# AVianEco/Softspoken

Measured on AMD Instinct MI355X. Metric: audio-seconds processed/sec (whole node), 16 kHz mono, higher is better.
Workload: dtype f16x2

## Files before the change

### softspoken_amd/build.py

```python
from __future__ import annotations

import os
import subprocess
import sys

HERE = os.path.dirname(os.path.abspath(__file__))
CSRC = os.path.join(HERE, "csrc")
OBJ = os.path.join(CSRC, "_obj")
LIB = os.path.join(HERE, "libsoftspoken_hip.so")
DEV_LIB = os.path.join(HERE, "libsoftspoken_hip_dev.so")
SOURCES = ["conv2.hip", "conv2_ups.hip", "conv4.hip", "conv4_ups.hip", "conv1s.hip", "frontend.hip", "heads.hip", "weights.hip", "engine.hip", "host.hip", "abi.hip", "stream.hip", "separate.hip"]
HEADERS = [os.path.join(CSRC, h) for h in ("kernels.h", "engine.h", "dsp.h", "mfma_util.h", "conv4_forms.h")] + [os.path.join(os.path.dirname(HERE), "include", "softspoken.h")]
FLAGS = ["-O3", "--offload-arch=gfx950", "-fPIC", "-std=c++17", "-Wno-unused-value"]
EXTRA_FLAGS = {"frontend.hip": ["-fno-slp-vectorize"], "conv4.hip": ["-fno-slp-vectorize"], "conv4_ups.hip": ["-fno-slp-vectorize"],
               "conv1s.hip": ["-fno-slp-vectorize"]}
DEV_SOURCES = ("conv2.hip", "conv2_ups.hip", "conv4.hip", "conv4_ups.hip", "conv1s.hip", "frontend.hip", "engine.hip", "weights.hip", "abi.hip", "separate.hip")
JITTER_LIB = DEV_LIB


def _hipcc():
    for cand in (os.environ.get("HIPCC"), "/opt/rocm/bin/hipcc"):
        if cand and os.path.exists(cand):
            return cand
    return "hipcc"


def _stale(target, deps):
    if not os.path.exists(target):
        return True
    t = os.path.getmtime(target)
# ... 36 lines not shown
```

### softspoken_amd/csrc/conv1s.hip

```cpp
#include "kernels.h"
#include "mfma_util.h"
#include <algorithm>
#include <type_traits>

namespace ss {

static constexpr int kH = 128, kW = 256, kC = 32;
static constexpr int kStrips = 9, kStripCols = 30;
static constexpr int kBank = 9 * 2 * 1024;
static constexpr int kS1Waves = 8;
static constexpr int kFPitch = 36;
static constexpr int kMaxRows = 32;
static constexpr int kFPatch = (kMaxRows + 5) * kFPitch;

__device__ __forceinline__ float s1_from_left(float v) {
    return __builtin_bit_cast(float, __builtin_amdgcn_update_dpp(0, __builtin_bit_cast(int, v), 0x138, 0xf, 0xf, true));
}
__device__ __forceinline__ float s1_from_right(float v) {
    return __builtin_bit_cast(float, __builtin_amdgcn_update_dpp(0, __builtin_bit_cast(int, v), 0x130, 0xf, 0xf, true));
}

struct S1Row { u32x4 f[2][2]; };

template <bool TRACK>
__global__ __launch_bounds__(64 * kS1Waves) __attribute__((amdgpu_waves_per_eu(2, 2)))
void conv1_stream_kernel(ConvArgs a, int rows_per_unit, int total_units) {
    extern __shared__ __attribute__((aligned(16))) char smem[];
// ... 258 lines not shown
        }
        if (k < rows_per_unit) {
            row_step(y0 + k, H0, H1, H2);
            if (k + 1 < rows_per_unit) row_step(y0 + k + 1, H1, H2, H0);
        }
    }
#ifdef SS_DEVBUILD
    if (a.stamps && lane == 0) {
        uint32_t* p = (uint32_t*)a.stamps + ((size_t)blockIdx.x * kS1Waves + wave) * 16;
        for (int i = 0; i < 7; ++i) p[i] = st_sum[i];
    }
#endif
    if (((ovf & 0x7fff7fffu) + 0x04000400u) & 0x80008000u) atomicOr(a.range_flag, 1);
}

struct S16Row { u32x4 f[2][2]; };

__device__ __forceinline__ f32x4 s16_mfma(const u32x4& a, const u32x4& b, const f32x4& c) {
    return __builtin_amdgcn_mfma_f32_16x16x32_f16(__builtin_bit_cast(f16x8, a), __builtin_bit_cast(f16x8, b), c, 0, 0, 0);
}
__device__ __forceinline__ int s16_shr1(int v) { return __builtin_amdgcn_update_dpp(0, v, 0x111, 0xf, 0xf, true); }
__device__ __forceinline__ int s16_shl1(int v) { return __builtin_amdgcn_update_dpp(0, v, 0x101, 0xf, 0xf, true); }
__device__ __forceinline__ float s16_shr1f(float v) { return __int_as_float(s16_shr1(__float_as_int(v))); }
__device__ __forceinline__ float s16_shl1f(float v) { return __int_as_float(s16_shl1(__float_as_int(v))); }

static constexpr int kFPatch16 = (kMaxRows + 6) * kFPitch;

template <bool TRACK>
__global__ __launch_bounds__(64 * kS1Waves) __attribute__((amdgpu_waves_per_eu(2, 2)))
void conv1_stream16_kernel(ConvArgs a, int rows_per_unit, int total_units) {
    extern __shared__ __attribute__((aligned(16))) char smem[];
    char* sW = smem;
    char* sK = smem + 2 * kBank;
    char* sPrev = sK + 4 * 1024;
    float* sF = (float*)(sPrev + kS1Waves * 2048);

    const int tid = threadIdx.x, lane = tid & 63, wave = __builtin_amdgcn_readfirstlane(tid >> 6);
    const int g = lane >> 4, c = lane & 15;
    for (int p = tid; p < 2 * kBank / 16; p += 64 * kS1Waves) *(u32x4*)(sW + p * 16) = *(const u32x4*)((const char*)a.wpk + (size_t)p * 16);
    u32x4 wf1[2];
// ... 126 lines not shown
                    Hn.f[t][0] = u32x4{ph[0][0], ph[0][1], ph[1][0], ph[1][1]};
                    Hn.f[t][1] = u32x4{pl[0][0], pl[0][1], pl[1][0], pl[1][1]};
                    if (edge_strip) {
#pragma unroll
                        for (int pq = 0; pq < 2; ++pq)
#pragma unroll
                            for (int e = 0; e < 4; ++e) Hn.f[t][pq][e] &= keep[t];
                    }
                }
            } else zero_row(Hn);
        };

        auto row_step = [&](int y, const S16Row& Ha, const S16Row& Hb, S16Row& Hn) {
            const float fc[2] = {fcen[0], fcen[1]};
            stamp(-1);
            u32x4 wh[2][2], wl[2][2];
            auto rd = [&](int tap) {
#pragma unroll
                for (int u = 0; u < 2; ++u) {
                    wh[tap & 1][u] = *(const u32x4*)(wl_base + (tap * 2 + u) * 1024);
                    wl[tap & 1][u] = *(const u32x4*)(wl_base + kBank + (tap * 2 + u) * 1024);
                }
            };
            const u32x4 kwl[2] = {*(const u32x4*)(sKl), *(const u32x4*)(sKl + 1024)};
            const u32x4 wrq[2] = {*(const u32x4*)(sKl + 2048), *(const u32x4*)(sKl + 3072)};
            rd(0);
            __builtin_amdgcn_sched_barrier(0);
            produce(y + 1, Hn, kwl);
            request(y + 2);
            stamp(1);
            f32x4 P[3][2][2];
#pragma unroll
            for (int t = 0; t < 2; ++t) {
                const uint32_t fh = pack_f16(fc[t], fc[t]);
                const uint32_t fl = split_lo(fh, fc[t], fc[t]);
                u32x4 bop = {(fh & 0xffffu) | (fl << 16), (fh & 0xffffu) | 0x3c000000u, 0x3c00u, 0u};
                if (g != 0) bop = u32x4{0u, 0u, 0u, 0u};
#pragma unroll
                for (int u = 0; u < 2; ++u) {
                    P[0][t][u] = f32x4{0.f, 0.f, 0.f, 0.f}; P[2][t][u] = f32x4{0.f, 0.f, 0.f, 0.f};
                    P[1][t][u] = s16_mfma(wrq[u], bop, f32x4{0.f, 0.f, 0.f, 0.f});
                }
            }
            __builtin_amdgcn_sched_barrier(0);
            stamp(4);
#pragma unroll
            for (int tap = 0; tap < 9; ++tap) {
                const int dy = tap / 3, dx = tap % 3;
                const S16Row& Hr = dy == 0 ? Ha : (dy == 1 ? Hb : Hn);
                if (tap + 1 < 9) rd(tap + 1);
                __builtin_amdgcn_sched_barrier(0);
#pragma unroll
                for (int pr = 0; pr < 3; ++pr)
#pragma unroll
                    for (int u = 0; u < 2; ++u)
#pragma unroll
                        for (int t = 0; t < 2; ++t)
                            P[dx][t][u] = s16_mfma(pr == 1 ? wl[tap & 1][u] : wh[tap & 1][u], Hr.f[t][pr == 0 ? 1 : 0], P[dx][t][u]);
                __builtin_amdgcn_sched_barrier(0);
            }
            __builtin_amdgcn_sched_barrier(0);
            stamp(0);
            float v[2][2][4];
#pragma unroll
            for (int u = 0; u < 2; ++u)
#pragma unroll
                for (int r = 0; r < 4; ++r) {
                    v[0][u][r] = relu_i(P[1][0][u][r] + s16_shr1f(P[0][1][u][r]) + P[2][1][u][r]);
                    v[1][u][r] = relu_i(P[1][1][u][r] + P[0][0][u][r] + s16_shl1f(P[2][0][u][r]));
                }
            auto store_px = [&](const float (&val)[2][4], char* dst, bool on, auto track_c) {
                constexpr bool track = TRACK && decltype(track_c)::value;
                uint32_t kh[4], kl[4];
#pragma unroll
                for (int i = 0; i < 4; ++i) {
                    const float e0 = val[i >> 1][2 * (i & 1)], e1 = val[i >> 1][2 * (i & 1) + 1];
                    kh[i] = pack_f16(e0, e1);
                    if (track) ovf = pk_max_u16(ovf, kh[i]);
                    kl[i] = split_lo(kh[i], e0, e1);
                }
                if (on) {
                    *(u32x4*)(dst) = u32x4{kh[0], kh[1], kh[2], kh[3]};
                    *(u32x4*)(dst + a.lo_delta) = u32x4{kl[0], kl[1], kl[2], kl[3]};
                }
            };
            f32x4 prv[2];
            if (y & 1) { prv[0] = *(const f32x4*)(prevp); prv[1] = *(const f32x4*)(prevp + 1024); }
            __builtin_amdgcn_sched_barrier(0);
#pragma unroll
            for (int t = 0; t < 2; ++t)
                store_px(v[t], (char*)a.out + (((size_t)n * kH + y) * kW + (size_t)max(xt[t], 0)) * (kC * 2) + g * 16, st_lane[t], std::true_type{});
            stamp(2);
            float cm[2][4];
#pragma unroll
// ... 87 lines not shown
```

### softspoken_amd/csrc/engine.h

```cpp
#pragma once
#include "../../include/softspoken.h"
#include "kernels.h"

#include <map>
#include <set>
#include <string>
#include <vector>

namespace ss {

inline size_t pcm_bytes_per_sample(int format) {
    switch (format) {
        case SS_PCM_U8: case SS_PCM_S8: return 1;
        case SS_PCM_S16: case SS_PCM_S16BE: return 2;
        case SS_PCM_S24: case SS_PCM_S24BE: return 3;
        case SS_PCM_F64: case SS_PCM_F64BE: return 8;
        default: return 4;
    }
}

int fail(ss_ctx* c, int code, const std::string& msg);
const char* thread_error();

#define HIPCHK(c, expr)                                                                                   \
// ... 12 lines not shown
    bool has(const std::string& k) const { return e.count(k) != 0; }
    const float* f32(const std::string& k, size_t count, std::string& err) const;
};
bool parse_blob(const void* p, size_t n, Blob& b, std::string& err);

enum Precision { kFp32 = 0, kBf16 = 1, kF16x2 = 2 };

struct ConvPlan {
    std::string name;
    void* d_w2 = nullptr; float* d_bias2 = nullptr; float* d_res_bias = nullptr; float* d_rank1 = nullptr;
    void* d_w3 = nullptr; void* d_proj = nullptr; float* d_bias3 = nullptr;
    void* d_w_ups = nullptr;
    bool s1_range_proven = false;
    void* d_w_s1 = nullptr;
    void* d_w_s16 = nullptr;
    void* d_w_upsr = nullptr;
    void* d_w_ups32 = nullptr;
    int ups32_nt = 1;
    int Cout = 0, NT = 1, C0 = 0, C1 = 0, R0 = 0, R1 = 0, H = 0, W = 0;
};

struct FileRec {
    int64_t off = 0;
    int64_t n = 0;
    int64_t n_padded = 0;
    double duration = 0;
    int64_t W = 0, win_base = 0;
    int64_t bin_off = 0; int n_bins = 0;
};

// ... 33 lines not shown
    ss::Precision prec = ss::kFp32;
    bool bf16 = false;
    bool profile = false, has_model = false;
    hipStream_t stream = nullptr;
    hipStream_t copy_stream = nullptr; hipEvent_t ev_copy = nullptr; bool copy_pending = false;
    std::string err;
    int chunk = 1024;
    double step = SS_STEP_DEFAULT;
    int num_cus = 256;

    float4* d_pretw = nullptr; float2* d_w2048 = nullptr;
    int *d_mel_start = nullptr, *d_mel_count = nullptr, *d_mel_off = nullptr; float* d_mel_w = nullptr; float* d_mel_wp = nullptr; int mel_nw = 0;
    float2 *d_win2 = nullptr, *d_twt = nullptr, *d_wkt = nullptr; float* d_mel_wq = nullptr; int* d_mel_p0 = nullptr;
    float *d_first_w = nullptr, *d_first_b = nullptr;
    float* d_flat_b = nullptr; void* d_flat_frag = nullptr; void* d_flat_frag4 = nullptr;
    float *d_spec_w = nullptr, *d_spec_b = nullptr;
    ss::Head1dWeights head{};
    std::vector<ss::ConvPlan> convs;
    std::vector<void*> owned;
    std::vector<void*> user_dev, user_host;

    unsigned long long *d_above = nullptr, *d_cov = nullptr, *h_above = nullptr, *h_cov = nullptr; size_t mask_cap = 0, cov_cap = 0, hmask_cap = 0;
    struct ResFile { int64_t W = 0, win_base = 0, bin_off = 0; int n_bins = 0; std::vector<ss_region> regions; };
    std::vector<ResFile> res_files; bool res_valid = false, res_regions = false; double res_thr = 0, res_brk = 0;
    unsigned long long *r_above = nullptr, *r_cov = nullptr; size_t rmask_cap = 0;
    uint64_t begin_gen = 0, res_gen = 0;
    std::vector<double> h_avg; std::vector<int32_t> h_cnt; bool avg_on_host = false; int64_t total_bins = 0;
    bool run_pending = false; double pend_thr = 0, pend_brk = 0; std::vector<ss::AvgFile> pend_af;
    double t_in = 0, t_plan = 0, t_sync = 0, t_loop = 0;
    std::vector<hipEvent_t> pass_ev; std::vector<int64_t> pass_done_at; size_t pass_reported = 0; int64_t progress_reported = 0, track_total = 0;
// ... 114 lines not shown
```

### softspoken_amd/csrc/engine.hip

```cpp
#include "engine.h"

#include <algorithm>
#include <chrono>
#include <cmath>
#include <cstdio>
#include <cstdlib>
#include <cstring>

namespace ss {

static thread_local std::string g_err;

int fail(ss_ctx* c, int code, const std::string& msg) {
    g_err = msg;
    if (c) c->err = msg;
    return code;
}
const char* thread_error() { return g_err.c_str(); }

double now_ms() { return std::chrono::duration<double, std::milli>(std::chrono::steady_clock::now().time_since_epoch()).count(); }

static int stat_id(ss_ctx* c, const std::string& name) {
    for (size_t i = 0; i < c->stats.size(); ++i) if (c->stats[i].name == name) return (int)i;
    KStat k; k.name = name; c->stats.push_back(k);
// ... 107 lines not shown
    Workspace& w = c->ws[1];
    if (w.chunk >= n) return true;
    if (!c->lane_stream) {
        if (hipStreamCreateWithFlags(&c->lane_stream, hipStreamNonBlocking) != hipSuccess) { c->lane_stream = nullptr; return false; }
        if (hipEventCreateWithFlags(&c->lane_ev_in, hipEventDisableTiming) != hipSuccess || hipEventCreateWithFlags(&c->lane_ev_out, hipEventDisableTiming) != hipSuccess) return false;
    }
    hipStreamSynchronize(c->lane_stream);
    free_ws(w);
    size_t free_b = 0, total_b = 0;
    if (hipMemGetInfo(&free_b, &total_b) != hipSuccess || (int64_t)free_b < c->ws[0].bytes + ((int64_t)4 << 30)) return false;
    std::string what;
    if (alloc_ws(c, n, c->lane_stream, w, what) != hipSuccess) { (void)hipGetLastError(); return false; }
    return true;
}

struct ConvExtra { const float* first_w = nullptr; const float* first_b = nullptr; const void* flat_w = nullptr; const void* flat_w4 = nullptr; float* flat_part = nullptr; int store_out = 1; };

static int base_dbg() {
    return (dev_env("SOFTSPOKEN_PRIO", 1) ? 32 : 0) | (dev_env("SOFTSPOKEN_ORDER", kOrderSideBySide ? 1 : 0) ? 512 : 0) | dev_env("SOFTSPOKEN_DBG", 0);
}

#ifdef SS_DEVBUILD
struct StageStamps {
    void* d_st = nullptr;
    static constexpr size_t st_bytes = (size_t)4096 * 8 * 16 * 4;
    int begin(ss_ctx* c, hipStream_t stream, const std::string& name, ConvArgs& a) {
        const char* want = getenv("SOFTSPOKEN_STAMP_LAYER");
        if (want && name == want) { HIPCHK(c, hipMalloc(&d_st, st_bytes)); HIPCHK(c, hipMemsetAsync(d_st, 0, st_bytes, stream)); a.stamps = d_st; }
        return SS_OK;
    }
    int end(ss_ctx* c, hipStream_t stream, const std::string& name, int n) {
// ... 137 lines not shown
    mark_written(c, ws, h); mark_written(c, ws, pool);
    if (ex.store_out) mark_written(c, ws, out);
    const double px = (double)n * pa.H * pa.W, cin = pa.C0 + pa.C1, cinb = pa.C0 + pa.C1 / 4.0;
    const double flops_a = 2.0 * px * pa.Cout * 9.0 * cin, bytes_a = px * es * (cinb + pa.Cout);
    auto v4 = [&](const ConvPlan& p, ConvArgs& x, double flops, double bytes) {
        return conv_launch(c, stream, conv_v4_variant(x, p.NT, cus, prec4), p.name, x, flops, bytes, -1.0,
                           [&](ConvArgs& y) { return launch_conv3x3_v4(y, p.NT, cus, prec4, stream); });
    };
    int rc;
    if (ups) {
        ScopedLaunch sl(c, stream, std::string(conv_ups_variant()) + "/" + pa.name, flops_a, bytes_a, px * pa.Cout * (9.0 * pa.C0 + 4.0 * pa.C1));
        HIPCHK(c, launch_conv3x3_ups(au, cus, stream));
    } else if ((rc = v4(pa, a, flops_a, bytes_a))) return rc;
    const double flops_b = 2.0 * px * pb.Cout * (9.0 * pb.Cout + cin) + (ex.flat_part ? 2.0 * px * 32 * 4 : 0.0);
    const double bytes_b = px * es * (pb.Cout + cinb + (ex.flat_part && !ex.store_out ? 0 : pb.Cout) + (pool ? pb.Cout / 4.0 : 0));
    if ((rc = v4(pb, b, flops_b, bytes_b))) return rc;
    if (ex.flat_part) ws.flat_groups = conv_v4_flat_groups();
    return SS_OK;
}

static int forward_chunk_(ss_ctx* c, Workspace& ws, hipStream_t stream, const float* signal, const int64_t* d_winoff, int n, float* d_logits, float* d_spec);

int forward_chunk(ss_ctx* c, Workspace& ws, hipStream_t stream, const float* signal, const int64_t* d_winoff, int n, float* d_logits, float* d_spec) {
#ifdef SS_DEVBUILD
    c->dbg_written.clear(); c->dbg_n = n; c->dbg_ws = (int)(&ws - c->ws);
    c->dbg_written.insert("feat");
    if (d_logits) c->dbg_written.insert("flat_part");
    const int rc = forward_chunk_(c, ws, stream, signal, d_winoff, n, d_logits, d_spec);
    if (rc) { c->dbg_written.clear(); c->dbg_n = 0; }
    return rc;
// ... 29 lines not shown
                        {"bott", nullptr, "he", "re", "enc", nullptr}, {"c4", "enc", "h6", "r6", "c6", nullptr},
                        {"c3", "c6", "h7", "r7", "c7", nullptr},   {"c2", "c7", "h8", "r8", "c8", nullptr}};
    const bool proj = c->prec != kFp32 && dev_env("SOFTSPOKEN_CONV4", 1) && dev_env("SOFTSPOKEN_RPROJ", 1);
    for (const Blk& b : blks) {
        if (proj) {
            rc = run_block_proj(c, ws, stream, cv[i], cv[i + 1], n, A(b.x0), b.x1 ? A(b.x1) : nullptr, A(b.h), A(b.y), b.pool ? A(b.pool) : nullptr);
            if (rc == SS_OK) { i += 2; continue; }
            if (rc != 1) return rc;
        }
        RC2(run_conv2(c, ws, stream, cv[i], n, A(b.x0), b.x1 ? A(b.x1) : nullptr, A(b.h), nullptr, A(b.r), nullptr, nullptr));
        RC2(run_conv2(c, ws, stream, cv[i + 1], n, A(b.h), nullptr, A(b.y), b.pool ? A(b.pool) : nullptr, nullptr, A(b.r), nullptr));
        i += 2;
    }
    {
        ConvExtra ex; ex.flat_w = c->d_flat_frag; ex.flat_w4 = c->d_flat_frag4; ex.flat_part = ws.flat; ex.store_out = d_spec ? 1 : 0;
        rc = 1;
        if (proj && (rc = run_block_proj(c, ws, stream, cv[i], cv[i + 1], n, A("c1"), A("c8"), A("h9"), A("c9"), nullptr, ex)) != 1) {
            if (rc) return rc;
        } else {
            RC2(run_conv2(c, ws, stream, cv[i], n, A("c1"), A("c8"), A("h9"), nullptr, A("r9"), nullptr, nullptr));
            RC2(run_conv2(c, ws, stream, cv[i + 1], n, A("h9"), nullptr, A("c9"), nullptr, nullptr, A("r9"), nullptr, ex));
        }
        i += 2;
    }
    if (d_spec) {
        RC2(run_conv2(c, ws, stream, cv[i], n, A("c9"), nullptr, A("hs"), nullptr, A("rs"), nullptr, nullptr));
        RC2(run_conv2(c, ws, stream, cv[i + 1], n, A("hs"), nullptr, A("s9"), nullptr, nullptr, A("rs"), nullptr));
        ScopedLaunch sl(c, stream, "spec_tail", 2.0 * n * 32768 * 64, (double)n * 32768 * (32 * es + 8));
        HIPCHK(c, launch_spec_tail(A("s9"), ws.lo_delta, c->d_spec_w, c->d_spec_b, d_spec, n, (int)c->prec, stream));
    }
// ... 333 lines not shown
```

### softspoken_amd/csrc/kernels.h

```cpp
#pragma once
#include <hip/hip_runtime.h>
#include <stdint.h>
#include <atomic>
#include <cstdlib>

namespace ss {

#ifdef SS_DEVBUILD
static inline int dev_env(const char* name, int dflt) { const char* v = getenv(name); return v ? atoi(v) : dflt; }
#else
static constexpr int dev_env(const char*, int dflt) { return dflt; }
#endif

inline hipError_t allow_full_lds(const void* kernel, std::atomic<uint64_t>& done) {
    int dev = 0;
    hipError_t e = hipGetDevice(&dev);
    if (e != hipSuccess) return e;
    const uint64_t bit = 1ull << (dev & 63);
    if (done.load(std::memory_order_acquire) & bit) return hipSuccess;
    e = hipFuncSetAttribute(kernel, hipFuncAttributeMaxDynamicSharedMemorySize, 160 * 1024);
    if (e == hipSuccess) done.fetch_or(bit, std::memory_order_release);
    return e;
}

// ... 94 lines not shown
bool conv_upsr_supports(const ConvArgs& a, int num_cus);
const char* conv_upsr_variant();
size_t conv_upsr_weight_bytes(int C0, int C1, int Cout);
hipError_t launch_conv3x3_upsr(const ConvArgs& a, int num_cus, hipStream_t s);

bool conv_ups32_supports(const ConvArgs& a, int NT, int MTW, int num_cus);
const char* conv_ups32_variant(int NT, int MTW);
size_t conv_ups32_weight_bytes(int C0, int C1, int Cout);
hipError_t launch_conv3x3_ups32(const ConvArgs& a, int NT, int MTW, int num_cus, hipStream_t s);

bool conv1_stream_supports(const ConvArgs& a);
const char* conv1_stream_variant(const ConvArgs& a, int form);
size_t conv1_stream_weight_bytes();
hipError_t launch_conv1_stream(const ConvArgs& a, int form, int rows_per_unit, int num_cus, hipStream_t s);

struct Head1dWeights { float w1[4][4][3], b1[4], w2[4][4][3], wr[4][4], b2r[4], wo[4], bo, fscale; };
hipError_t launch_mask_head_parts(const float* parts, int n_parts, const float* flat_bias, const Head1dWeights& hw, float* logits,
                                  int N, hipStream_t s);
hipError_t launch_spec_tail(const void* x, int64_t lo_delta, const float* w , const float* bias, float* spec, int N, int prec,
                            hipStream_t s);

static constexpr int kMelLo = 10, kMelHi = 32, kMelPitch = 43;
struct FrontendTables {
    const float4* pretw;
    const float2* w2048;
    const int* mel_start;
    const int* mel_count;
    const int* mel_off;
    const float* mel_w;
    int mel_nw;
// ... 58 lines not shown
```

### softspoken_amd/csrc/weights.hip

```cpp
#include "engine.h"

#include <algorithm>
#include <cmath>
#include <cstring>

namespace ss {

const float* Blob::f32(const std::string& k, size_t count, std::string& err) const {
    auto it = e.find(k);
    if (it == e.end()) { err = "weights blob: missing tensor '" + k + "'"; return nullptr; }
    if (it->second.dtype != 0 || it->second.nbytes != count * 4) {
        err = "weights blob: tensor '" + k + "' has wrong dtype/size"; return nullptr;
    }
    return (const float*)(base + it->second.offset);
}

bool parse_blob(const void* p, size_t n, Blob& b, std::string& err) {
    if (n < 16 || memcmp(p, "SSWBLOB1", 8) != 0) { err = "weights blob: bad magic"; return false; }
    uint32_t cnt; memcpy(&cnt, (const char*)p + 8, 4);
    if (16 + (size_t)cnt * sizeof(BlobEntry) > n) { err = "weights blob: truncated table"; return false; }
    b.base = (const char*)p; b.size = n;
    for (uint32_t i = 0; i < cnt; ++i) {
        BlobEntry en; memcpy(&en, (const char*)p + 16 + (size_t)i * sizeof(BlobEntry), sizeof(BlobEntry));
        en.name[95] = 0;
// ... 127 lines not shown

static void pack_conv_stream16(const Folded& w3, std::vector<char>& out, bool& range_ok) {
    const size_t bank = (size_t)9 * 2 * 1024;
    out.assign(2 * bank, 0);
    for (int t = 0; t < 9; ++t)
        for (int u = 0; u < 2; ++u)
            for (int l = 0; l < 64; ++l)
                for (int j = 0; j < 8; ++j) {
                    const int i = l & 15, g = l >> 4, co = 8 * (i >> 2) + 4 * u + (i & 3), ci = 8 * g + j;
                    const float v = w3.w[((size_t)co * w3.cin + ci) * 9 + t];
                    const uint16_t hi = f2h(v), lo = f2h(v - h2f(hi));
                    if ((hi & 0x7c00u) == 0x7c00u) range_ok = false;
                    const size_t off = ((size_t)(t * 2 + u) * 64 + l) * 16 + (size_t)j * 2;
                    memcpy(&out[off], &hi, 2); memcpy(&out[off + bank], &lo, 2);
                }
}

static void pack_conv_split_ups(const Folded& w3, int c0, int c1, std::vector<char>& out, bool& range_ok) {
    const size_t bank_r = (size_t)9 * 2048, bank_u = (size_t)16 * 2048;
    const int nreg = c0 / 32, nups = c1 / 32;
    out.assign((size_t)nreg * 2 * bank_r + (size_t)nups * 2 * bank_u, 0);
    auto put = [&](size_t off_hi, size_t off_lo, float v) {
        const uint16_t hi = f2h(v), lo = f2h(v - h2f(hi));
        if ((hi & 0x7c00u) == 0x7c00u) range_ok = false;
        memcpy(&out[off_hi], &hi, 2); memcpy(&out[off_lo], &lo, 2);
    };
    for (int ci = 0; ci < nreg; ++ci)
        for (int t = 0; t < 9; ++t)
            for (int s = 0; s < 2; ++s)
                for (int l = 0; l < 64; ++l)
// ... 369 lines not shown
        if ((rc = dev_upload(c, &B.d_bias3, b2r.data(), cout * 4))) return rc;
    }
    if (c->prec == kF16x2 && cin % 16 == 0) {
        const int steps = cin / 16, tiles = cout / 32;
        const size_t bank = (size_t)steps * tiles * 64 * 8;
        std::vector<uint16_t> pj(2 * bank);
        for (int st = 0; st < steps; ++st) for (int t = 0; t < tiles; ++t) for (int l = 0; l < 64; ++l) for (int j = 0; j < 8; ++j) {
            const float v = fr.w[(size_t)(32 * t + (l & 31)) * cin + 16 * st + 8 * (l >> 5) + j];
            const uint16_t hi = f2h(v);
            if ((hi & 0x7c00u) == 0x7c00u) c->split_range_ok = false;
            const size_t at = (((size_t)st * tiles + t) * 64 + l) * 8 + j;
            pj[at] = hi; pj[bank + at] = f2h(v - h2f(hi));
        }
        if ((rc = dev_upload(c, (char**)&B.d_proj, (const char*)pj.data(), pj.size() * 2))) return rc;
        if ((rc = dev_upload(c, &B.d_bias3, b2r.data(), cout * 4))) return rc;
    }
    if (c->prec == kF16x2) pack_conv_split(f2, nullptr, NTB, pk, c->split_range_ok); else pack_conv_v2(f2, nullptr, c->bf16, NT, pk);
    if ((rc = dev_upload(c, (char**)&B.d_w2, pk.data(), pk.size()))) return rc;
    if ((rc = dev_upload(c, &B.d_bias2, f2.b.data(), cout * 4))) return rc;
    c->convs.push_back(B);
    return SS_OK;
}

int build_model(ss_ctx* c, const Blob& bl) {
    int rc;
    c->split_range_ok = true;
    struct RB { const char* n; int c0, c1, co, H, W; const char *x0, *x1, *h, *y, *pool; };
    const RB rbs[] = {{"conv1_1", 1, 0, 32, 128, 256, nullptr, nullptr, "h1", "c1", "p1"},
                      {"conv2_1", 32, 0, 64, 64, 128, "conv1_1", nullptr, "h2", "c2", "p2"},
                      {"conv3_1", 64, 0, 96, 32, 64, "conv2_1", nullptr, "h3", "c3", "p3"},
// ... 61 lines not shown
        if ((rc = dev_upload(c, (char**)&c->d_flat_frag4, (const char*)t4.data(), t4.size() * 2))) return rc;
    }
    if (c->prec == kF16x2) {
        const size_t bank = (size_t)64 * 2 * 64 * 8;
        std::vector<uint16_t> t4(2 * bank, 0);
        for (int pr = 0; pr < 64; ++pr) for (int s2 = 0; s2 < 2; ++s2) for (int l = 0; l < 64; ++l) for (int j = 0; j < 8; ++j) {
            const int row = l & 31, ch = 16 * s2 + 8 * (j >> 2) + 4 * (l >> 5) + (j & 3);
            if (row >= 8) continue;
            const float v = wf[((size_t)(row & 3) * 32 + ch) * 128 + 2 * pr + (row >> 2)];
            const uint16_t hi = f2h(v);
            if ((hi & 0x7c00u) == 0x7c00u) c->split_range_ok = false;
            const size_t at = (((size_t)pr * 2 + s2) * 64 + l) * 8 + j;
            t4[at] = hi; t4[bank + at] = f2h(v - h2f(hi));
        }
        if ((rc = dev_upload(c, (char**)&c->d_flat_frag4, (const char*)t4.data(), t4.size() * 2))) return rc;
    }
    if ((rc = dev_upload(c, &c->d_flat_b, bf, 16))) return rc;
    const float* ws = bl.f32("spec_output_conv.1.weight", 64, err);
    const float* bs = bl.f32("spec_output_conv.1.bias", 2, err);
    if (!ws || !bs) return fail(c, SS_ERR_FORMAT, err);
    float wss[64];
    for (int co = 0; co < 2; ++co) for (int ci = 0; ci < 32; ++ci) wss[co * 32 + ci] = std::ldexp(ws[co * 32 + ci], -sc["spec_output_conv.0"][ci]);
    if ((rc = dev_upload(c, &c->d_spec_w, wss, 256))) return rc;
    if ((rc = dev_upload(c, &c->d_spec_b, bs, 8))) return rc;
    Folded f1, f2, fr;
    const std::string p = "mask_output_conv.0";
    if (!fold_conv_bn(bl, p + ".conv1.0", p + ".conv1.1", 4, 4, 3, f1, err)) return fail(c, SS_ERR_FORMAT, err);
    if (!fold_conv_bn(bl, p + ".conv2.0", p + ".conv2.1", 4, 4, 3, f2, err)) return fail(c, SS_ERR_FORMAT, err);
    if (!fold_conv_bn(bl, p + ".residual.0", p + ".residual.1", 4, 4, 1, fr, err)) return fail(c, SS_ERR_FORMAT, err);
    const float* wo = bl.f32("mask_output_conv.1.weight", 4, err);
// ... 22 lines not shown
```

Baseline: 32210.

## Add fused streaming 3x3 conv kernel with residual projection and flat head

Adds a conv9 streaming f16x2 kernel for the 32-channel 128x256 block that fuses the 1x1 residual projection of two inputs, the 3x3 conv, ReLU, and the flattening-head partial reduction into one row-streaming pass. It reuses the conv1 stream16 tap loop, which is factored into a shared header. The goal is to avoid separate launches and the intermediate activation round trips to memory for this block. In exchange it needs new packed weight layouts and more LDS and register pressure, and the engine only uses it when the shape checks pass.

Result: faster. 33150, median of 6 (+2.9%).

```diff
diff --git a/softspoken_amd/build.py b/softspoken_amd/build.py
--- a/softspoken_amd/build.py
+++ b/softspoken_amd/build.py
@@ -9,11 +9,11 @@
 OBJ = os.path.join(CSRC, "_obj")
 LIB = os.path.join(HERE, "libsoftspoken_hip.so")
 DEV_LIB = os.path.join(HERE, "libsoftspoken_hip_dev.so")
-SOURCES = ["conv2.hip", "conv2_ups.hip", "conv4.hip", "conv4_ups.hip", "conv1s.hip", "frontend.hip", "heads.hip", "weights.hip", "engine.hip", "host.hip", "abi.hip", "stream.hip", "separate.hip"]
-HEADERS = [os.path.join(CSRC, h) for h in ("kernels.h", "engine.h", "dsp.h", "mfma_util.h", "conv4_forms.h")] + [os.path.join(os.path.dirname(HERE), "include", "softspoken.h")]
+SOURCES = ["conv2.hip", "conv2_ups.hip", "conv4.hip", "conv4_ups.hip", "conv1s.hip", "conv9s.hip", "frontend.hip", "heads.hip", "weights.hip", "engine.hip", "host.hip", "abi.hip", "stream.hip", "separate.hip"]
+HEADERS = [os.path.join(CSRC, h) for h in ("kernels.h", "engine.h", "dsp.h", "mfma_util.h", "conv4_forms.h", "stream16.h")] + [os.path.join(os.path.dirname(HERE), "include", "softspoken.h")]
 FLAGS = ["-O3", "--offload-arch=gfx950", "-fPIC", "-std=c++17", "-Wno-unused-value"]
 EXTRA_FLAGS = {"frontend.hip": ["-fno-slp-vectorize"], "conv4.hip": ["-fno-slp-vectorize"], "conv4_ups.hip": ["-fno-slp-vectorize"],
-               "conv1s.hip": ["-fno-slp-vectorize"]}
+               "conv1s.hip": ["-fno-slp-vectorize"], "conv9s.hip": ["-fno-slp-vectorize"]}
 DEV_SOURCES = ("conv2.hip", "conv2_ups.hip", "conv4.hip", "conv4_ups.hip", "conv1s.hip", "frontend.hip", "engine.hip", "weights.hip", "abi.hip", "separate.hip")
 JITTER_LIB = DEV_LIB
 
diff --git a/softspoken_amd/csrc/conv1s.hip b/softspoken_amd/csrc/conv1s.hip
--- a/softspoken_amd/csrc/conv1s.hip
+++ b/softspoken_amd/csrc/conv1s.hip
@@ -1,16 +1,11 @@
 #include "kernels.h"
-#include "mfma_util.h"
+#include "stream16.h"
 #include <algorithm>
 #include <type_traits>
 
 namespace ss {
 
-static constexpr int kH = 128, kW = 256, kC = 32;
-static constexpr int kStrips = 9, kStripCols = 30;
-static constexpr int kBank = 9 * 2 * 1024;
-static constexpr int kS1Waves = 8;
 static constexpr int kFPitch = 36;
-static constexpr int kMaxRows = 32;
 static constexpr int kFPatch = (kMaxRows + 5) * kFPitch;
 
 __device__ __forceinline__ float s1_from_left(float v) {
@@ -299,16 +294,6 @@
     if (((ovf & 0x7fff7fffu) + 0x04000400u) & 0x80008000u) atomicOr(a.range_flag, 1);
 }
 
-struct S16Row { u32x4 f[2][2]; };
-
-__device__ __forceinline__ f32x4 s16_mfma(const u32x4& a, const u32x4& b, const f32x4& c) {
-    return __builtin_amdgcn_mfma_f32_16x16x32_f16(__builtin_bit_cast(f16x8, a), __builtin_bit_cast(f16x8, b), c, 0, 0, 0);
-}
-__device__ __forceinline__ int s16_shr1(int v) { return __builtin_amdgcn_update_dpp(0, v, 0x111, 0xf, 0xf, true); }
-__device__ __forceinline__ int s16_shl1(int v) { return __builtin_amdgcn_update_dpp(0, v, 0x101, 0xf, 0xf, true); }
-__device__ __forceinline__ float s16_shr1f(float v) { return __int_as_float(s16_shr1(__float_as_int(v))); }
-__device__ __forceinline__ float s16_shl1f(float v) { return __int_as_float(s16_shl1(__float_as_int(v))); }
-
 static constexpr int kFPatch16 = (kMaxRows + 6) * kFPitch;
 
 template <bool TRACK>
@@ -465,17 +450,10 @@
         auto row_step = [&](int y, const S16Row& Ha, const S16Row& Hb, S16Row& Hn) {
             const float fc[2] = {fcen[0], fcen[1]};
             stamp(-1);
-            u32x4 wh[2][2], wl[2][2];
-            auto rd = [&](int tap) {
-#pragma unroll
-                for (int u = 0; u < 2; ++u) {
-                    wh[tap & 1][u] = *(const u32x4*)(wl_base + (tap * 2 + u) * 1024);
-                    wl[tap & 1][u] = *(const u32x4*)(wl_base + kBank + (tap * 2 + u) * 1024);
-                }
-            };
+            S16Ring ring;
             const u32x4 kwl[2] = {*(const u32x4*)(sKl), *(const u32x4*)(sKl + 1024)};
             const u32x4 wrq[2] = {*(const u32x4*)(sKl + 2048), *(const u32x4*)(sKl + 3072)};
-            rd(0);
+            ring.rd(wl_base, 0);
             __builtin_amdgcn_sched_barrier(0);
             produce(y + 1, Hn, kwl);
             request(y + 2);
@@ -495,40 +473,17 @@
             }
             __builtin_amdgcn_sched_barrier(0);
             stamp(4);
-#pragma unroll
-            for (int tap = 0; tap < 9; ++tap) {
-                const int dy = tap / 3, dx = tap % 3;
-                const S16Row& Hr = dy == 0 ? Ha : (dy == 1 ? Hb : Hn);
-                if (tap + 1 < 9) rd(tap + 1);
-                __builtin_amdgcn_sched_barrier(0);
-#pragma unroll
-                for (int pr = 0; pr < 3; ++pr)
-#pragma unroll
-                    for (int u = 0; u < 2; ++u)
-#pragma unroll
-                        for (int t = 0; t < 2; ++t)
-                            P[dx][t][u] = s16_mfma(pr == 1 ? wl[tap & 1][u] : wh[tap & 1][u], Hr.f[t][pr == 0 ? 1 : 0], P[dx][t][u]);
-                __builtin_amdgcn_sched_barrier(0);
-            }
-            __builtin_amdgcn_sched_barrier(0);
+            s16_taps(ring, wl_base, Ha, Hb, Hn, P, [](int) {});
             stamp(0);
             float v[2][2][4];
-#pragma unroll
-            for (int u = 0; u < 2; ++u)
-#pragma unroll
-                for (int r = 0; r < 4; ++r) {
-                    v[0][u][r] = relu_i(P[1][0][u][r] + s16_shr1f(P[0][1][u][r]) + P[2][1][u][r]);
-                    v[1][u][r] = relu_i(P[1][1][u][r] + P[0][0][u][r] + s16_shl1f(P[2][0][u][r]));
-                }
+            s16_combine(P, v);
             auto store_px = [&](const float (&val)[2][4], char* dst, bool on, auto track_c) {
                 constexpr bool track = TRACK && decltype(track_c)::value;
                 uint32_t kh[4], kl[4];
-#pragma unroll
-                for (int i = 0; i < 4; ++i) {
-                    const float e0 = val[i >> 1][2 * (i & 1)], e1 = val[i >> 1][2 * (i & 1) + 1];
-                    kh[i] = pack_f16(e0, e1);
-                    if (track) ovf = pk_max_u16(ovf, kh[i]);
-                    kl[i] = split_lo(kh[i], e0, e1);
+                s16_split_px(val, kh, kl);
+                if (track) {
+#pragma unroll
+                    for (int i = 0; i < 4; ++i) ovf = pk_max_u16(ovf, kh[i]);
                 }
                 if (on) {
                     *(u32x4*)(dst) = u32x4{kh[0], kh[1], kh[2], kh[3]};
diff --git a/softspoken_amd/csrc/conv9s.hip b/softspoken_amd/csrc/conv9s.hip
--- /dev/null
+++ b/softspoken_amd/csrc/conv9s.hip
@@ -0,0 +1,195 @@
+#include "kernels.h"
+#include "stream16.h"
+#include <algorithm>
+
+namespace ss {
+
+static constexpr int kProjFrag = 2 * 2 * 2 * 1024;
+static constexpr uint32_t kRowB = kW * 64, kRowB8 = (kW / 2) * 64;
+
+__global__ __launch_bounds__(64 * kS1Waves) __attribute__((amdgpu_waves_per_eu(2, 2)))
+void conv9_stream16_kernel(ConvArgs a, int rows_per_unit, int total_units) {
+    extern __shared__ __attribute__((aligned(16))) char smem[];
+    char* sW = smem;
+    char* sP = smem + 2 * kBank;
+
+    const int tid = threadIdx.x, lane = tid & 63, wave = __builtin_amdgcn_readfirstlane(tid >> 6);
+    const int g = lane >> 4, c = lane & 15;
+    for (int p = tid; p < 2 * kBank / 16; p += 64 * kS1Waves) *(u32x4*)(sW + p * 16) = *(const u32x4*)((const char*)a.wpk + (size_t)p * 16);
+    for (int p = tid; p < kProjFrag / 16; p += 64 * kS1Waves) *(u32x4*)(sP + p * 16) = *(const u32x4*)((const char*)a.proj_w + (size_t)p * 16);
+    const f32x4 bias[2] = {*(const f32x4*)(a.bias + 8 * g), *(const f32x4*)(a.bias + 8 * g + 4)};
+    __syncthreads();
+
+    const char* wl_base = sW + lane * 16;
+    const char* pl_base = sP + lane * 16;
+    const char* fw_base = (const char*)a.flat_w4 + lane * 16;
+    const int bands = kH / rows_per_unit;
+    const int64_t lo = a.lo_delta;
+    uint32_t ovf = 0;
+
+    for (int unit = (int)blockIdx.x * kS1Waves + wave; unit < total_units; unit += (int)gridDim.x * kS1Waves) {
+        const int s = unit % kStrips, b = (unit / kStrips) % bands, n = unit / (kStrips * bands);
+        const int x0 = kStripCols * s - 1, y0 = b * rows_per_unit, ylast = y0 + rows_per_unit - 1;
+        uint32_t keep[2], voff[2]; bool st_lane[2];
+        int xt[2];
+#pragma unroll
+        for (int t = 0; t < 2; ++t) {
+            const int mm = 2 * c + t;
+            xt[t] = x0 + mm;
+            keep[t] = (unsigned)xt[t] < (unsigned)kW ? 0xffffffffu : 0u;
+            st_lane[t] = mm >= 1 && mm <= kStripCols && xt[t] < kW;
+            voff[t] = (uint32_t)min(max(xt[t], 0), kW - 1) * 64u + (uint32_t)g * 16u;
+        }
+        const uint32_t voff8 = (uint32_t)(min(max(xt[1], 0), kW - 1) >> 1) * 64u + (uint32_t)g * 16u;
+        const char* hw = (const char*)a.src0 + (size_t)n * kH * kRowB;
+        const char* c1w = (const char*)a.xp0 + (size_t)n * kH * kRowB;
+        const char* c8w = (const char*)a.xp1 + (size_t)n * (kH / 2) * kRowB8;
+        char* ow = (char*)a.out + (size_t)n * kH * kRowB;
+
+        auto load_row = [&](S16Row& H, int r) {
+            const char* p = hw + (size_t)min(max(r, 0), kH - 1) * kRowB;
+#pragma unroll
+            for (int t = 0; t < 2; ++t) { H.f[t][0] = *(const u32x4*)(p + voff[t]); H.f[t][1] = *(const u32x4*)(p + lo + voff[t]); }
+        };
+        auto mask_row = [&](S16Row& H, int r) {
+            const uint32_t rk = (unsigned)r < (unsigned)kH ? 0xffffffffu : 0u;
+#pragma unroll
+            for (int t = 0; t < 2; ++t)
+#pragma unroll
+                for (int pq = 0; pq < 2; ++pq)
+#pragma unroll
+                    for (int e = 0; e < 4; ++e) H.f[t][pq][e] &= keep[t] & rk;
+        };
+        S16Row H0, H1, H2;
+        S16Row C1;
+        u32x4 C8[2];
+        auto load_c1 = [&](int r) {
+            const char* p = c1w + (size_t)r * kRowB;
+#pragma unroll
+            for (int t = 0; t < 2; ++t) { C1.f[t][0] = *(const u32x4*)(p + voff[t]); C1.f[t][1] = *(const u32x4*)(p + lo + voff[t]); }
+        };
+        auto load_c8 = [&](int r8) {
+            const char* p = c8w + (size_t)r8 * kRowB8;
+            C8[0] = *(const u32x4*)(p + voff8); C8[1] = *(const u32x4*)(p + lo + voff8);
+        };
+        f32x4 F[2] = {f32x4{0.f, 0.f, 0.f, 0.f}, f32x4{0.f, 0.f, 0.f, 0.f}};
+        uint32_t ovt[2] = {0u, 0u};
+
+        auto row_step = [&](int y, S16Row& Ha, const S16Row& Hb, S16Row& Hn) {
+            S16Ring ring;
+            ring.rd(wl_base, 0);
+            u32x4 pw[2][2][2];
+#pragma unroll
+            for (int q = 0; q < 8; ++q) pw[q >> 2][(q >> 1) & 1][q & 1] = *(const u32x4*)(pl_base + q * 1024);
+            const u32x4 fwh = *(const u32x4*)(fw_base + (size_t)(2 * y) * 1024), fwl = *(const u32x4*)(fw_base + (size_t)(2 * y + 1) * 1024);
+            __builtin_amdgcn_sched_barrier(0);
+            f32x4 P[3][2][2];
+#pragma unroll
+            for (int t = 0; t < 2; ++t)
+#pragma unroll
+                for (int u = 0; u < 2; ++u) { P[0][t][u] = f32x4{0.f, 0.f, 0.f, 0.f}; P[1][t][u] = bias[u]; P[2][t][u] = f32x4{0.f, 0.f, 0.f, 0.f}; }
+            u32x4 c8t0[2];
+#pragma unroll
+            for (int pq = 0; pq < 2; ++pq)
+#pragma unroll
+                for (int e = 0; e < 4; ++e) c8t0[pq][e] = (uint32_t)s16_shr1((int)C8[pq][e]);
+#pragma unroll
+            for (int src = 0; src < 2; ++src)
+#pragma unroll
+                for (int pr = 0; pr < 3; ++pr)
+#pragma unroll
+                    for (int u = 0; u < 2; ++u)
+#pragma unroll
+                        for (int t = 0; t < 2; ++t) {
+                            const int pq = pr == 0 ? 1 : 0;
+                            const u32x4& x = src == 0 ? C1.f[t][pq] : (t ? C8[pq] : c8t0[pq]);
+                            P[1][t][u] = s16_mfma(pw[src][u][pr == 1 ? 1 : 0], x, P[1][t][u]);
+                        }
+            __builtin_amdgcn_sched_barrier(0);
+            load_c1(min(y + 1, ylast));
+            load_c8(min(y + 1, ylast) >> 1);
+            __builtin_amdgcn_sched_barrier(0);
+            s16_taps(ring, wl_base, Ha, Hb, Hn, P, [&](int tap) {
+                if (tap == 2) load_row(Ha, min(y + 2, ylast + 1));
+                if (tap == 5) mask_row(Hn, y + 1);
+            });
+            float v[2][2][4];
+            s16_combine(P, v);
+            uint32_t kh[2][4], kl[2][4];
+#pragma unroll
+            for (int t = 0; t < 2; ++t) {
+                s16_split_px(v[t], kh[t], kl[t]);
+#pragma unroll
+                for (int i = 0; i < 4; ++i) ovt[t] = pk_max_u16(ovt[t], kh[t][i]);
+            }
+#pragma unroll
+            for (int pr = 0; pr < 3; ++pr)
+#pragma unroll
+                for (int t = 0; t < 2; ++t) {
+                    const uint32_t (&k)[4] = pr == 0 ? kl[t] : kh[t];
+                    F[t] = s16_mfma(pr == 1 ? fwl : fwh, u32x4{k[0], k[1], k[2], k[3]}, F[t]);
+                }
+            if (a.store_out) {
+                char* p = ow + (size_t)y * kRowB;
+#pragma unroll
+                for (int t = 0; t < 2; ++t)
+                    if (st_lane[t]) {
+                        *(u32x4*)(p + voff[t]) = u32x4{kh[t][0], kh[t][1], kh[t][2], kh[t][3]};
+                        *(u32x4*)(p + lo + voff[t]) = u32x4{kl[t][0], kl[t][1], kl[t][2], kl[t][3]};
+                    }
+            }
+        };
+
+        load_row(H0, y0 - 1); load_row(H1, y0); load_c1(y0); load_c8(y0 >> 1); load_row(H2, y0 + 1);
+        mask_row(H0, y0 - 1); mask_row(H1, y0);
+        int k = 0;
+        for (; k + 3 <= rows_per_unit; k += 3) {
+            row_step(y0 + k, H0, H1, H2);
+            row_step(y0 + k + 1, H1, H2, H0);
+            row_step(y0 + k + 2, H2, H0, H1);
+        }
+        if (k < rows_per_unit) {
+            row_step(y0 + k, H0, H1, H2);
+            if (k + 1 < rows_per_unit) row_step(y0 + k + 1, H1, H2, H0);
+        }
+#pragma unroll
+        for (int t = 0; t < 2; ++t) {
+            if (g == 0 && st_lane[t]) {
+                float* fp = a.flat_part + ((size_t)n * bands + b) * 4 * kW + xt[t];
+#pragma unroll
+                for (int r = 0; r < 4; ++r) fp[r * kW] = F[t][r];
+            }
+            if (st_lane[t]) ovf = pk_max_u16(ovf, ovt[t]);
+        }
+    }
+    if (((ovf & 0x7fff7fffu) + 0x04000400u) & 0x80008000u) atomicOr(a.range_flag, 1);
+}
+
+static bool px64(ActStride s) { return s.pix == 64u; }
+bool conv9_stream_supports(const ConvArgs& a) {
+    return a.H == kH && a.W == kW && a.Cout == kC && a.C0 == kC && a.C1 == 0 && a.C0x == kC && a.C1x == kC && a.src0 && a.xp0 && a.xp1 && a.wpk &&
+           a.proj_w && a.bias && a.flat_w4 && a.flat_part && (a.out || !a.store_out) && !a.pool_out && !a.res_in && a.lo_delta != 0 && a.range_flag &&
+           a.N > 0 && px64(a.s_src0) && px64(a.s_xp0) && px64(a.s_xp1) && (px64(a.s_out) || !a.store_out);
+}
+const char* conv9_stream_variant() { return "conv9_stream16_kernel"; }
+size_t conv9_stream_proj_bytes() { return kProjFrag; }
+size_t conv9_stream_flat_bytes() { return (size_t)kH * 2 * 1024; }
+bool conv9_stream_rows_ok(int rows_per_unit) { return rows_per_unit >= 2 && !(rows_per_unit & 1) && kH % rows_per_unit == 0 && rows_per_unit <= kMaxRows; }
+int conv9_stream_flat_groups(int rows_per_unit) { return kH / rows_per_unit; }
+double conv9_stream_issued_macs(int N) { return (double)N * kH * kStrips * ((24 + 108 + 6) / 3) * (16.0 * 16 * 32); }
+
+hipError_t launch_conv9_stream(const ConvArgs& a, int rows_per_unit, int grid_override, int num_cus, hipStream_t s) {
+    if (!conv9_stream_supports(a) || !conv9_stream_rows_ok(rows_per_unit)) return hipErrorInvalidValue;
+    const int64_t total = (int64_t)a.N * (kH / rows_per_unit) * kStrips;
+    if (total >= (int64_t)1 << 30) return hipErrorInvalidValue;
+    const int cus = num_cus > 0 ? num_cus : 256;
+    int grid = (int)std::min<int64_t>(cus, (total + kS1Waves - 1) / kS1Waves);
+    if (grid_override > 0) grid = std::min(grid, grid_override);
+    static std::atomic<uint64_t> attr_done{0};
+    const size_t lds = 2 * (size_t)kBank + kProjFrag;
+    if (hipError_t e = allow_full_lds((const void*)conv9_stream16_kernel, attr_done)) return e;
+    hipLaunchKernelGGL(conv9_stream16_kernel, dim3(grid), dim3(64 * kS1Waves), lds, s, a, rows_per_unit, (int)total);
+    return hipGetLastError();
+}
+
+}
diff --git a/softspoken_amd/csrc/engine.h b/softspoken_amd/csrc/engine.h
--- a/softspoken_amd/csrc/engine.h
+++ b/softspoken_amd/csrc/engine.h
@@ -50,6 +50,7 @@
     bool s1_range_proven = false;
     void* d_w_s1 = nullptr;
     void* d_w_s16 = nullptr;
+    void* d_proj_s16 = nullptr;
     void* d_w_upsr = nullptr;
     void* d_w_ups32 = nullptr;
     int ups32_nt = 1;
@@ -113,6 +114,7 @@
     float2 *d_win2 = nullptr, *d_twt = nullptr, *d_wkt = nullptr; float* d_mel_wq = nullptr; int* d_mel_p0 = nullptr;
     float *d_first_w = nullptr, *d_first_b = nullptr;
     float* d_flat_b = nullptr; void* d_flat_frag = nullptr; void* d_flat_frag4 = nullptr;
+    void* d_flat_rows = nullptr;
     float *d_spec_w = nullptr, *d_spec_b = nullptr;
     ss::Head1dWeights head{};
     std::vector<ss::ConvPlan> convs;
diff --git a/softspoken_amd/csrc/engine.hip b/softspoken_amd/csrc/engine.hip
--- a/softspoken_amd/csrc/engine.hip
+++ b/softspoken_amd/csrc/engine.hip
@@ -145,7 +145,8 @@
     return true;
 }
 
-struct ConvExtra { const float* first_w = nullptr; const float* first_b = nullptr; const void* flat_w = nullptr; const void* flat_w4 = nullptr; float* flat_part = nullptr; int store_out = 1; };
+struct ConvExtra { const float* first_w = nullptr; const float* first_b = nullptr; const void* flat_w = nullptr; const void* flat_w4 = nullptr; float* flat_part = nullptr; int store_out = 1;
+                   const void* flat_rows = nullptr; };
 
 static int base_dbg() {
     return (dev_env("SOFTSPOKEN_PRIO", 1) ? 32 : 0) | (dev_env("SOFTSPOKEN_ORDER", kOrderSideBySide ? 1 : 0) ? 512 : 0) | dev_env("SOFTSPOKEN_DBG", 0);
@@ -313,6 +314,19 @@
     } else if ((rc = v4(pa, a, flops_a, bytes_a))) return rc;
     const double flops_b = 2.0 * px * pb.Cout * (9.0 * pb.Cout + cin) + (ex.flat_part ? 2.0 * px * 32 * 4 : 0.0);
     const double bytes_b = px * es * (pb.Cout + cinb + (ex.flat_part && !ex.store_out ? 0 : pb.Cout) + (pool ? pb.Cout / 4.0 : 0));
+    if (c->prec == kF16x2 && ex.flat_part && ex.flat_rows && pb.d_w_s16 && pb.d_proj_s16 && dev_env("SOFTSPOKEN_C9S", 1)) {
+        ConvArgs bs = b;
+        bs.wpk = pb.d_w_s16; bs.proj_w = pb.d_proj_s16; bs.flat_w4 = ex.flat_rows;
+        const int rows = dev_env("SOFTSPOKEN_C9S_ROWS", 32);
+        if (conv9_stream_supports(bs) && conv9_stream_rows_ok(rows)) {
+            const int grid = dev_env("SOFTSPOKEN_C9S_GRID", 0);
+            if ((rc = conv_launch(c, stream, conv9_stream_variant(), pb.name, bs, flops_b, bytes_b, conv9_stream_issued_macs(n),
+                                  [&](ConvArgs& y) { return launch_conv9_stream(y, rows, grid, cus, stream); })))
+                return rc;
+            ws.flat_groups = conv9_stream_flat_groups(rows);
+            return SS_OK;
+        }
+    }
     if ((rc = v4(pb, b, flops_b, bytes_b))) return rc;
     if (ex.flat_part) ws.flat_groups = conv_v4_flat_groups();
     return SS_OK;
@@ -372,6 +386,7 @@
     }
     {
         ConvExtra ex; ex.flat_w = c->d_flat_frag; ex.flat_w4 = c->d_flat_frag4; ex.flat_part = ws.flat; ex.store_out = d_spec ? 1 : 0;
+        ex.flat_rows = c->d_flat_rows;
         rc = 1;
         if (proj && (rc = run_block_proj(c, ws, stream, cv[i], cv[i + 1], n, A("c1"), A("c8"), A("h9"), A("c9"), nullptr, ex)) != 1) {
             if (rc) return rc;
diff --git a/softspoken_amd/csrc/kernels.h b/softspoken_amd/csrc/kernels.h
--- a/softspoken_amd/csrc/kernels.h
+++ b/softspoken_amd/csrc/kernels.h
@@ -132,6 +132,15 @@
 size_t conv1_stream_weight_bytes();
 hipError_t launch_conv1_stream(const ConvArgs& a, int form, int rows_per_unit, int num_cus, hipStream_t s);
 
+bool conv9_stream_supports(const ConvArgs& a);
+const char* conv9_stream_variant();
+size_t conv9_stream_proj_bytes();
+size_t conv9_stream_flat_bytes();
+bool conv9_stream_rows_ok(int rows_per_unit);
+int conv9_stream_flat_groups(int rows_per_unit);
+double conv9_stream_issued_macs(int N);
+hipError_t launch_conv9_stream(const ConvArgs& a, int rows_per_unit, int grid_override, int num_cus, hipStream_t s);
+
 struct Head1dWeights { float w1[4][4][3], b1[4], w2[4][4][3], wr[4][4], b2r[4], wo[4], bo, fscale; };
 hipError_t launch_mask_head_parts(const float* parts, int n_parts, const float* flat_bias, const Head1dWeights& hw, float* logits,
                                   int N, hipStream_t s);
diff --git a/softspoken_amd/csrc/stream16.h b/softspoken_amd/csrc/stream16.h
--- /dev/null
+++ b/softspoken_amd/csrc/stream16.h
@@ -0,0 +1,74 @@
+#pragma once
+#include "mfma_util.h"
+
+namespace ss {
+
+static constexpr int kH = 128, kW = 256, kC = 32;
+static constexpr int kStrips = 9, kStripCols = 30;
+static constexpr int kBank = 9 * 2 * 1024;
+static constexpr int kS1Waves = 8;
+static constexpr int kMaxRows = 32;
+
+struct S16Row { u32x4 f[2][2]; };
+
+__device__ __forceinline__ f32x4 s16_mfma(const u32x4& a, const u32x4& b, const f32x4& c) {
+    return __builtin_amdgcn_mfma_f32_16x16x32_f16(__builtin_bit_cast(f16x8, a), __builtin_bit_cast(f16x8, b), c, 0, 0, 0);
+}
+__device__ __forceinline__ int s16_shr1(int v) { return __builtin_amdgcn_update_dpp(0, v, 0x111, 0xf, 0xf, true); }
+__device__ __forceinline__ int s16_shl1(int v) { return __builtin_amdgcn_update_dpp(0, v, 0x101, 0xf, 0xf, true); }
+__device__ __forceinline__ float s16_shr1f(float v) { return __int_as_float(s16_shr1(__float_as_int(v))); }
+__device__ __forceinline__ float s16_shl1f(float v) { return __int_as_float(s16_shl1(__float_as_int(v))); }
+
+struct S16Ring {
+    u32x4 wh[2][2], wl[2][2];
+    __device__ __forceinline__ void rd(const char* wl_base, int tap) {
+#pragma unroll
+        for (int u = 0; u < 2; ++u) {
+            wh[tap & 1][u] = *(const u32x4*)(wl_base + (tap * 2 + u) * 1024);
+            wl[tap & 1][u] = *(const u32x4*)(wl_base + kBank + (tap * 2 + u) * 1024);
+        }
+    }
+};
+
+template <typename AfterTap>
+__device__ __forceinline__ void s16_taps(S16Ring& ring, const char* wl_base, const S16Row& Ha, const S16Row& Hb, const S16Row& Hn, f32x4 (&P)[3][2][2],
+                                         AfterTap&& after_tap) {
+#pragma unroll
+    for (int tap = 0; tap < 9; ++tap) {
+        const int dy = tap / 3, dx = tap % 3;
+        const S16Row& Hr = dy == 0 ? Ha : (dy == 1 ? Hb : Hn);
+        if (tap + 1 < 9) ring.rd(wl_base, tap + 1);
+        __builtin_amdgcn_sched_barrier(0);
+#pragma unroll
+        for (int pr = 0; pr < 3; ++pr)
+#pragma unroll
+            for (int u = 0; u < 2; ++u)
+#pragma unroll
+                for (int t = 0; t < 2; ++t)
+                    P[dx][t][u] = s16_mfma(pr == 1 ? ring.wl[tap & 1][u] : ring.wh[tap & 1][u], Hr.f[t][pr == 0 ? 1 : 0], P[dx][t][u]);
+        __builtin_amdgcn_sched_barrier(0);
+        if (tap + 1 < 9) after_tap(tap);
+    }
+    __builtin_amdgcn_sched_barrier(0);
+}
+
+__device__ __forceinline__ void s16_combine(const f32x4 (&P)[3][2][2], float (&v)[2][2][4]) {
+#pragma unroll
+    for (int u = 0; u < 2; ++u)
+#pragma unroll
+        for (int r = 0; r < 4; ++r) {
+            v[0][u][r] = relu_i(P[1][0][u][r] + s16_shr1f(P[0][1][u][r]) + P[2][1][u][r]);
+            v[1][u][r] = relu_i(P[1][1][u][r] + P[0][0][u][r] + s16_shl1f(P[2][0][u][r]));
+        }
+}
+
+__device__ __forceinline__ void s16_split_px(const float (&val)[2][4], uint32_t (&kh)[4], uint32_t (&kl)[4]) {
+#pragma unroll
+    for (int i = 0; i < 4; ++i) {
+        const float e0 = val[i >> 1][2 * (i & 1)], e1 = val[i >> 1][2 * (i & 1) + 1];
+        kh[i] = pack_f16(e0, e1);
+        kl[i] = split_lo(kh[i], e0, e1);
+    }
+}
+
+}
diff --git a/softspoken_amd/csrc/weights.hip b/softspoken_amd/csrc/weights.hip
--- a/softspoken_amd/csrc/weights.hip
+++ b/softspoken_amd/csrc/weights.hip
@@ -165,6 +165,36 @@
                     const size_t off = ((size_t)(t * 2 + u) * 64 + l) * 16 + (size_t)j * 2;
                     memcpy(&out[off], &hi, 2); memcpy(&out[off + bank], &lo, 2);
                 }
+}
+
+static void pack_proj_stream16(const Folded& wr, std::vector<char>& out, bool& range_ok) {
+    out.assign((size_t)2 * 2 * 2 * 1024, 0);
+    for (int src = 0; src < 2; ++src)
+        for (int u = 0; u < 2; ++u)
+            for (int l = 0; l < 64; ++l)
+                for (int j = 0; j < 8; ++j) {
+                    const int i = l & 15, co = 8 * (i >> 2) + 4 * u + (i & 3), ci = 32 * src + 8 * (l >> 4) + j;
+                    const float v = wr.w[(size_t)co * wr.cin + ci];
+                    const uint16_t hi = f2h(v), lo = f2h(v - h2f(hi));
+                    if ((hi & 0x7c00u) == 0x7c00u) range_ok = false;
+                    const size_t off = ((size_t)((src * 2 + u) * 2) * 64 + l) * 16 + (size_t)j * 2;
+                    memcpy(&out[off], &hi, 2); memcpy(&out[off + 1024], &lo, 2);
+                }
+}
+
+static void pack_flat_rows(const float* wf, std::vector<char>& out, bool& range_ok) {
+    out.assign((size_t)128 * 2 * 1024, 0);
+    for (int h = 0; h < 128; ++h)
+        for (int l = 0; l < 64; ++l)
+            for (int j = 0; j < 8; ++j) {
+                const int row = l & 15, ch = 8 * (l >> 4) + j;
+                if (row >= 4) continue;
+                const float v = wf[((size_t)row * 32 + ch) * 128 + h];
+                const uint16_t hi = f2h(v), lo = f2h(v - h2f(hi));
+                if ((hi & 0x7c00u) == 0x7c00u) range_ok = false;
+                const size_t off = ((size_t)(h * 2) * 64 + l) * 16 + (size_t)j * 2;
+                memcpy(&out[off], &hi, 2); memcpy(&out[off + 1024], &lo, 2);
+            }
 }
 
 static void pack_conv_split_ups(const Folded& w3, int c0, int c1, std::vector<char>& out, bool& range_ok) {
@@ -564,6 +594,14 @@
         }
         if ((rc = dev_upload(c, (char**)&B.d_proj, (const char*)pj.data(), pj.size() * 2))) return rc;
         if ((rc = dev_upload(c, &B.d_bias3, b2r.data(), cout * 4))) return rc;
+        if (cin0 == 32 && cin1 == 32 && cout == 32 && H == 128 && W == 256) {
+            pack_conv_stream16(f2, pk, c->split_range_ok);
+            if (pk.size() != conv1_stream_weight_bytes()) return fail(c, SS_ERR_STATE, "pack_conv_stream16: size");
+            if ((rc = dev_upload(c, (char**)&B.d_w_s16, pk.data(), pk.size()))) return rc;
+            pack_proj_stream16(fr, pk, c->split_range_ok);
+            if (pk.size() != conv9_stream_proj_bytes()) return fail(c, SS_ERR_STATE, "pack_proj_stream16: size");
+            if ((rc = dev_upload(c, (char**)&B.d_proj_s16, pk.data(), pk.size()))) return rc;
+        }
     }
     if (c->prec == kF16x2) pack_conv_split(f2, nullptr, NTB, pk, c->split_range_ok); else pack_conv_v2(f2, nullptr, c->bf16, NT, pk);
     if ((rc = dev_upload(c, (char**)&B.d_w2, pk.data(), pk.size()))) return rc;
@@ -655,6 +693,10 @@
             t4[at] = hi; t4[bank + at] = f2h(v - h2f(hi));
         }
         if ((rc = dev_upload(c, (char**)&c->d_flat_frag4, (const char*)t4.data(), t4.size() * 2))) return rc;
+        std::vector<char> rows;
+        pack_flat_rows(wf, rows, c->split_range_ok);
+        if (rows.size() != conv9_stream_flat_bytes()) return fail(c, SS_ERR_STATE, "pack_flat_rows: size");
+        if ((rc = dev_upload(c, (char**)&c->d_flat_rows, rows.data(), rows.size()))) return rc;
     }
     if ((rc = dev_upload(c, &c->d_flat_b, bf, 16))) return rc;
     const float* ws = bl.f32("spec_output_conv.1.weight", 64, err);
```
